# JunweiLiang/Multiverse

Measured on AMD Instinct MI355X. Metric: trajectories/sec (8-obs/12-pred, multi-scale 18x32+9x16 grid, greedy forward), higher is better.
Workload: dtype f16x3 (fp32 operands as two pre-scaled fp16 planes, fp32 accumulate and state; winograd F(3,3) over image rows on pre-transformed operands, 1.67 fp16 MFMAs issued per fp32 product over the gate kernels; error vs fp64 within 2x of the fp32-MFMA path's -- asserted under checkpoint-like dynamic range (; 1 GPU; BASELINE configs[1]: multi-scale 18x32+9x16 (scene 36x64x11), batch 64/GPU, fp32 forward-only, beam 1, obs 8 / pred 12; gate convolution on the fp16 matrix pipe (f16x3 split, fp32-class error); batch_per_gpu=64, global_batch=64, obs_len=8, pred_len=12, parallelism=batch-sharded x1, no data-path collective

## Files before the change

multiverse_amd/csrc/convlstm_mfma.h:

```cpp
#pragma once
#include <hip/hip_runtime.h>
#include <stdint.h>

#include <vector>

namespace mv {

typedef float f32x16 __attribute__((ext_vector_type(16)));
typedef float f32x4 __attribute__((ext_vector_type(4)));

constexpr int kBN = 128;
constexpr int kBK = 32;
constexpr int kChBlock = 32;
constexpr int kWaveRows = 32;
constexpr int kBlockRows = 128;
constexpr int kMaxGroup = 4;

struct ConvLstmArgs {
  const float* x;
  const float* h;
  const float* c;
  const int32_t* src_row_h;
  const int32_t* src_row_c;
  const float* wpack;
  const float* bias;
  float* h_out;
  float* c_out;
  float* gates_out;
  float* out0;
  float* out1;
  int32_t out0_cols, out1_cols;
  int32_t n_colblocks;
  int32_t ng_last;
  int32_t rows, H, W, Cx, C;
  int32_t x_row_stride;
  int32_t n_xchunks;
  int32_t n_hchunks;
  int32_t w_chunks;
  int32_t x_small;
  int32_t zero_state;
  float forget_bias;
  int32_t want_h16;
  int32_t skip_h32;
  const float* sx_bias;
  const float* sx_corr;
  const int32_t* sx_hot;
  const uint32_t* sx_cellyx;
  int32_t sx_hot_stride, sx_hot_div, sx_rad, sx_by_class;
  const int32_t* cone_list;
  const int32_t* cone_prev;
  int32_t cone_on;
  int32_t cone_cells;
};

struct ConvLstmGroup {
  ConvLstmArgs p[kMaxGroup];
  int32_t block_end[kMaxGroup];
  int32_t n;
};

static inline int convlstm_xchunks(int Cx) {
  if (Cx == 0) return 0;
  if (9 * Cx <= kBK) return 1;
  return 9 * (Cx / kBK);
}
static inline bool convlstm_cx_supported(int Cx) {
  return Cx == 0 || 9 * Cx <= kBK || (Cx % kBK) == 0;
}
static inline size_t convlstm_wpack_elems(int Cx, int C) {
  const size_t nch = (size_t)convlstm_xchunks(Cx) + 9 * (size_t)(C / kBK);
  return (size_t)(C / kChBlock) * nch * kBN * kBK;
}

static inline void pack_convlstm_weights(const float* w, int Cx, int C, float* out) {
  const int Cin = Cx + C, N4 = 4 * C;
  const int nx = convlstm_xchunks(Cx), nh = 9 * (C / kBK), nch = nx + nh;
  const bool small = (Cx > 0 && 9 * Cx <= kBK);
  for (int cb = 0; cb < C / kChBlock; ++cb)
    for (int q = 0; q < nch; ++q) {
      float* tile = out + ((size_t)cb * nch + q) * kBN * kBK;
      for (int kk = 0; kk < 4; ++kk)
        for (int g = 0; g < 4; ++g)
          for (int l = 0; l < 64; ++l)
            for (int j = 0; j < 4; ++j) {
              const int k = kk * 8 + (l >> 5) * 4 + j;
              const int n = g * C + cb * kChBlock + (l & 31);
              int tap = -1, ci = -1;
              if (q < nx) {
                if (small) {
                  if (k < 9 * Cx) { tap = k / Cx; ci = k % Cx; }
                } else {
                  tap = q % 9; ci = (q / 9) * kBK + k;
                }
              } else {
                const int qq = q - nx;
                tap = qq % 9; ci = Cx + (qq / 9) * kBK + k;
              }
              tile[((kk * 4 + g) * 64 + l) * 4 + j] =
                  (tap < 0) ? 0.f : w[((size_t)tap * Cin + ci) * N4 + n];
            }
    }
}

__device__ __forceinline__ float sigm_(float v) {
  const float e = __builtin_amdgcn_exp2f(-1.4426950408889634f * v);
// ... 301 lines not shown
```

multiverse_amd/csrc/convlstm_wino3.h:

```cpp
#pragma once
#include "convlstm_wino.h"

namespace mv {

template <int NRB>
struct Wn3 {
  static constexpr int kCh = 8 * NRB;
  static constexpr int kChunkVec = 5 * 3 * 2 * NRB * 64;
  static constexpr uint32_t kChunkBytes = kChunkVec * 16;
  static constexpr int kTileFloats = 96 * kCh;
};

static inline size_t wino3_wpack_elems(int Cx16, int C, int nrb) {
  return (size_t)(C / (8 * nrb)) * (size_t)(Cx16 / 16 + C / 16) * 5 * 3 * 2 * nrb * 64 * 8;
}

__global__ void pack_wino3_kernel(const float* __restrict__ w, _Float16* __restrict__ out,
                                  int Cx_total, int Cx16, int C, int nrb, size_t total) {
  const size_t idx = (size_t)blockIdx.x * blockDim.x + threadIdx.x;
  if (idx >= total) return;
  const int e = idx & 7;
  const int l = (idx >> 3) & 63;
  size_t t = idx >> 9;
  const int rb = (int)(t % nrb); t /= nrb;
// ... 15 lines not shown
  switch (comp) {
    case 0: u = 0.5 * g0; break;
    case 1: u = -0.5 * (g0 + g1 + g2); break;
    case 2: u = (-g0 + g1 - g2) / 6.0; break;
    case 3: u = (g0 + 2.0 * g1 + 4.0 * g2) / 6.0; break;
    default: u = -g2; break;
  }
  const double sv = u * 256.0;
  note_pack_range(sv);
  const _Float16 v0 = (_Float16)sv;
  const _Float16 v1 = (_Float16)(sv - (double)v0);
  const size_t vec = ((((size_t)cb * nch + chunk) * 5 + comp) * 3 + dx) * 2;
  out[(((vec + 0) * nrb + rb) * 64 + l) * 8 + e] = v0;
  out[(((vec + 1) * nrb + rb) * 64 + l) * 8 + e] = v1;
}

struct Wn3Consts { f16x8 m1, p2, m2; };

template <int KA, int KB>
__device__ __forceinline__ void wn_lin(const f16x8 a_hi, const f16x8 a_lo, const f16x8 b_hi,
                                       const f16x8 b_lo, const Wn3Consts& k, f16x8& hi,
                                       f16x8& lo) {
  static_assert((KA == 1 && (KB == 1 || KB == -1 || KB == -2)) || (KA == 2 && KB == 1), "form");
  const f16x8 nka = KA == 1 ? k.m1 : k.m2;
  f16x8 s, ne2, l1;
  if (KA == 2) {
    s = __builtin_elementwise_fma(a_hi, k.p2, b_hi);
    l1 = __builtin_elementwise_fma(a_lo, k.p2, b_lo);
  } else if (KB == 1) {
    s = a_hi + b_hi;
    l1 = a_lo + b_lo;
  } else {
    s = __builtin_elementwise_fma(b_hi, KB == -1 ? k.m1 : k.m2, a_hi);
    l1 = __builtin_elementwise_fma(b_lo, KB == -1 ? k.m1 : k.m2, a_lo);
  }
  const f16x8 bb = __builtin_elementwise_fma(a_hi, nka, s);
  const f16x8 t = __builtin_elementwise_fma(bb, k.m1, s);
  const f16x8 ne1 = __builtin_elementwise_fma(a_hi, nka, t);
  if (KB == -1) ne2 = bb + b_hi;
  else ne2 = __builtin_elementwise_fma(b_hi, KB == 1 ? k.m1 : k.p2, bb);
  hi = s;
  lo = __builtin_elementwise_fma(ne1 + ne2, k.m1, l1);
}

struct Wn3TransformItem {
  const _Float16* p0;
  int64_t pstride;
  _Float16* out;
  const int32_t* src_row;
  int32_t rows, H, W, Cc;
  const int32_t* cone_list;
  const int32_t* cone_prev;
  int32_t cone_cells;
};
constexpr int kW3TrGroup = 8;
struct Wn3TransformGroup {
  Wn3TransformItem it[kW3TrGroup];
  int32_t blk_end[kW3TrGroup];
  int32_t n;
};
static inline size_t wino3_v_elems(int rows, int H, int W, int Cc) {
  const size_t Q = (size_t)rows * ((H + 2) / 3) * W;
  return ((Q + 31) / 32) * (size_t)(Cc / 16) * 5 * 2 * 64 * 8;
}
static inline unsigned wino3_transform_blocks(int rows, int H, int W, int Cc) {
  const size_t Q = (size_t)rows * ((H + 2) / 3) * W;
  return (unsigned)((((Q + 31) / 32) * (size_t)(Cc / 16) + 3) / 4);
}
__global__ __launch_bounds__(256)
void wino3_transform_kernel(const Wn3TransformGroup g) {
  int block = blockIdx.x, pi = 0;
#pragma unroll
  for (int i = 0; i < kW3TrGroup - 1; ++i)
    if (i + 1 < g.n && (int)blockIdx.x >= g.blk_end[i]) pi = i + 1;
  if (pi > 0) block -= g.blk_end[pi - 1];
  const Wn3TransformItem& it = g.it[pi];
  const int lane = threadIdx.x & 63, wave = threadIdx.x >> 6;
  const int KG = it.Cc >> 4;
  const int H = it.H, W = it.W, HW = H * W;
  const int Kt = ((H + 2) / 3) * W, Q_total = it.rows * Kt;
  const int ntile = (Q_total + 31) >> 5;
  const int wid = block * 4 + wave;
  if (wid >= ntile * KG) return;
  int tile = wid / KG;
  const int cg = wid - tile * KG;
  if (it.cone_list) {
    if (tile >= it.cone_list[0]) return;
    tile = it.cone_list[4 + tile];
  }
  const int col = lane & 31, half = lane >> 5;
  const int q = tile * 32 + col;
  const bool valid = q < Q_total;
  int r = 0, y0 = 0, xpos = 0;
  if (valid) {
    r = q / Kt;
    const int pc = q - r * Kt;
    const int t = pc / W;
    y0 = 3 * t;
    xpos = pc - t * W;
  }
  const int sr = (valid && it.src_row) ? it.src_row[r] : r;
  int sr_up = sr, sr_mid = sr, sr_dn = sr;
  if (it.cone_prev && valid) {
    const int bg = it.rows - 1;
    const int* prev = it.cone_prev;
    sr_mid = prev[q >> 5] ? sr : bg;
    sr_up = (y0 > 0 && !prev[(q - W) >> 5]) ? bg : sr;
    sr_dn = (y0 + 3 < H && !prev[(q + W) >> 5]) ? bg : sr;
  }
  f16x8 dh[5], dl[5];
#pragma unroll
  for (int i = 0; i < 5; ++i) {
    const int rho = y0 - 1 + i;
    const bool ok = valid & (rho >= 0) & (rho < H);
    const long long m = (long long)(i == 0 ? sr_up : (i == 4 ? sr_dn : sr_mid)) * HW + rho * W + xpos;
    const size_t o = ((size_t)(m >> 5) * KG + cg) * 512 + (size_t)(half * 256 + (int)(m & 31) * 8);
    const f16x8 z = {0, 0, 0, 0, 0, 0, 0, 0};
    dh[i] = ok ? *reinterpret_cast<const f16x8*>(it.p0 + o) : z;
    dl[i] = ok ? *reinterpret_cast<const f16x8*>(it.p0 + it.pstride + o) : z;
  }
  uint32_t mone = 0xBC00BC00u, ptwo = 0x40004000u, mtwo = 0xC000C000u;
  asm volatile("" : "+s"(mone), "+s"(ptwo), "+s"(mtwo));
  Wn3Consts kc;
  kc.m1 = __builtin_bit_cast(f16x8, u32x4{mone, mone, mone, mone});
  kc.p2 = __builtin_bit_cast(f16x8, u32x4{ptwo, ptwo, ptwo, ptwo});
  kc.m2 = __builtin_bit_cast(f16x8, u32x4{mtwo, mtwo, mtwo, mtwo});
  f16x8 vh[5], vl[5], th, tl, t3h, t3l;
  wn_lin<1, -1>(dh[3], dl[3], dh[1], dl[1], kc, vh[3], vl[3]);
  wn_lin<1, -1>(dh[0], dl[0], dh[2], dl[2], kc, th, tl);
  wn_lin<2, 1>(th, tl, vh[3], vl[3], kc, vh[0], vl[0]);
  wn_lin<1, -1>(dh[3], dl[3], dh[2], dl[2], kc, t3h, t3l);
  wn_lin<1, -2>(t3h, t3l, dh[1], dl[1], kc, vh[1], vl[1]);
  wn_lin<1, -1>(dh[1], dl[1], dh[2], dl[2], kc, th, tl);
  wn_lin<2, 1>(th, tl, t3h, t3l, kc, vh[2], vl[2]);
  wn_lin<1, -1>(dh[2], dl[2], dh[4], dl[4], kc, th, tl);
  wn_lin<2, 1>(vh[3], vl[3], th, tl, kc, vh[4], vl[4]);
  f16x8* o = reinterpret_cast<f16x8*>(it.out) + ((size_t)tile * KG + cg) * (5 * 2 * 64) + lane;
#pragma unroll
  for (int c = 0; c < 5; ++c) {
    o[(c * 2 + 0) * 64] = vh[c];
    o[(c * 2 + 1) * 64] = vl[c];
  }
}
static inline void launch_wino3_transforms(const Wn3TransformItem* items, int n,
                                           hipStream_t stream) {
  for (int i0 = 0; i0 < n; i0 += kW3TrGroup) {
    Wn3TransformGroup g{};
    g.n = n - i0 < kW3TrGroup ? n - i0 : kW3TrGroup;
    unsigned nb = 0;
    for (int j = 0; j < g.n; ++j) {
      g.it[j] = items[i0 + j];
      nb += wino3_transform_blocks(g.it[j].rows, g.it[j].H, g.it[j].W, g.it[j].Cc);
      g.blk_end[j] = (int32_t)nb;
    }
    for (int j = g.n; j < kW3TrGroup; ++j) g.blk_end[j] = (int32_t)nb;
    if (nb) hipLaunchKernelGGL(wino3_transform_kernel, dim3(nb), dim3(256), 0, stream, g);
  }
}

template <int WAVES, int NRB, bool HALO, bool BF16D = false>
__device__ __forceinline__ void convlstm_wino3_body(const ConvLstmWinoArgs& p, int cb, int mt,
                                                    f16x8* lds) {
  using G = Wn3<NRB>;
  constexpr int CH = G::kCh;
  constexpr int kOwn = HALO ? 30 : 32;
  constexpr int kTriples = WAVES * kOwn;
  constexpr int kPieces = CH / 4;
  constexpr int kPasses = (96 * kPieces + 63) / 64;
  const ConvLstm16Args& q = p.b;
  const ConvLstmArgs& a = q.f;
  const int tid = threadIdx.x;
  const int lane = tid & 63;
// ... 371 lines not shown
        }
#pragma unroll
        for (int g = 0; g < 4; ++g)
          add[g] = *reinterpret_cast<const f32x4*>(bsrc + g * C + ch);
        if (a.sx_corr) {
          const int dy = y - hot_y, dxh = xpos - hot_x, rad = a.sx_rad;
          const bool inr = okc[e] && !bg_row && dy >= -rad && dy <= rad && dxh >= -rad && dxh <= rad;
          const int dyc = dy < -rad ? -rad : (dy > rad ? rad : dy);
          const int dxc = dxh < -rad ? -rad : (dxh > rad ? rad : dxh);
          const int side = 2 * rad + 1;
          const int idx = a.sx_by_class
                              ? 3 * (hot_y == 0 ? 0 : (hot_y == H - 1 ? 2 : 1)) +
                                    (hot_x == 0 ? 0 : (hot_x == W - 1 ? 2 : 1))
                              : ((valid && !bg_row) ? r : 0);
          const float* ct = a.sx_corr +
              ((size_t)idx * side * side + (dyc + rad) * side + (dxc + rad)) * 4 * C + ch;
          const float keep = inr ? 1.0f : 0.0f;
#pragma unroll
          for (int g = 0; g < 4; ++g) {
            const f32x4 cv = *reinterpret_cast<const f32x4*>(ct + g * C);
            add[g][0] = __builtin_fmaf(cv[0], keep, add[g][0]);
            add[g][1] = __builtin_fmaf(cv[1], keep, add[g][1]);
            add[g][2] = __builtin_fmaf(cv[2], keep, add[g][2]);
            add[g][3] = __builtin_fmaf(cv[3], keep, add[g][3]);
          }
        }
      }
      f32x4 cn4, hn4, si4, tj4, sf4, so4;
#pragma unroll
      for (int j = 0; j < 4; ++j) {
        float pre[4];
#pragma unroll
        for (int g = 0; g < 4; ++g) {
          const int reg = g * 4 + j;
          float yv;
          if constexpr (BF16D) {
            yv = acc[e][rb][reg];
          } else {
            const float m0 = acc[0][rb][reg], m1 = acc[1][rb][reg], m2 = acc[2][rb][reg],
                        m3 = acc[3][rb][reg], m4 = acc[kAcc - 1][rb][reg];
            if (e == 0) yv = (m0 + m1) + (m2 + m3);
            else if (e == 1) yv = (m1 - m2) + 2.0f * m3;
            else yv = (m1 + m2) + (4.0f * m3 + m4);
          }
          pre[g] = __builtin_fmaf(yv, un, add[g][j]);
        }
        const float si = sigm_(pre[0]), tj = tanh_(pre[1]), sf = sigm_(pre[2] + a.forget_bias),
                    so = sigm_(pre[3]);
        float cn = sf * cprev[e][rb][j];
        cn = cn + si * tj;
        const float hn = tanh_(cn) * so;
        cn4[j] = cn; hn4[j] = hn; si4[j] = si; tj4[j] = tj; sf4[j] = sf; so4[j] = so;
      }
      *reinterpret_cast<f32x4*>(tl0 + wr_idx + e * 32 * CH + rb * 8) = cn4;
      if (!a.skip_h32) *reinterpret_cast<f32x4*>(tl1 + wr_idx + e * 32 * CH + rb * 8) = hn4;
      if (a.gates_out && okc[e]) {
        const uint32_t g0 = (mcell * 4u * (uint32_t)C + (uint32_t)ch) * 4u;
        __builtin_amdgcn_raw_buffer_store_b128(__builtin_bit_cast(u32x4, si4), go_rs, (int)g0,
                                               0, MV_EPI_ST_AUX);
        __builtin_amdgcn_raw_buffer_store_b128(__builtin_bit_cast(u32x4, tj4), go_rs,
                                               (int)(g0 + rowb), 0, MV_EPI_ST_AUX);
        __builtin_amdgcn_raw_buffer_store_b128(__builtin_bit_cast(u32x4, sf4), go_rs,
                                               (int)(g0 + 2 * rowb), 0, MV_EPI_ST_AUX);
        __builtin_amdgcn_raw_buffer_store_b128(__builtin_bit_cast(u32x4, so4), go_rs,
                                               (int)(g0 + 3 * rowb), 0, MV_EPI_ST_AUX);
      }
      if (planes) {
        f16x4 p0, p1;
#pragma unroll
        for (int j = 0; j < 4; ++j) {
          if constexpr (BF16D) {
            p0[j] = bf16_as_half(hn4[j]);
            p1[j] = p0[j];
          } else {
            const float sc = hn4[j] * kF16Scale;
            const _Float16 h0 = (_Float16)sc;
            p0[j] = h0;
            p1[j] = (_Float16)(sc - (float)h0);
          }
        }
        ph[e][rb] = __builtin_bit_cast(u32x2, p0);
        pl[e][rb] = __builtin_bit_cast(u32x2, p1);
      }
    }
  }
  asm volatile("s_waitcnt lgkmcnt(0)" ::: "memory");
  {
#pragma unroll
    for (int k = 0; k < kPasses; ++k) {
      const int i = k * 64 + lane_e;
      const int trow = i / kPieces, piece = i - trow * kPieces;
      if (96 * kPieces % 64 == 0 || trow < 96) {
        const uint32_t ro = otab[96 + trow];
        const u32x4 cv = *reinterpret_cast<const u32x4*>(tl0 + i * 4);
        u32x4 hv = cv;
        if (!a.skip_h32) hv = *reinterpret_cast<const u32x4*>(tl1 + i * 4);
        if (ro != kNone) {
          const int off = (int)(ro + colb + (uint32_t)piece * 16u);
          __builtin_amdgcn_raw_buffer_store_b128(cv, co_rs, off, 0, MV_EPI_ST_AUX);
          if (!a.skip_h32) __builtin_amdgcn_raw_buffer_store_b128(hv, ho_rs, off, 0, MV_EPI_ST_AUX);
        }
      }
    }
  }
  if (planes) {
    const uint32_t mc01 = (uint32_t)(r * HW + (half_e ? cell[1] : cell[0]));
    const uint32_t mc2 = (uint32_t)(r * HW + cell[2]);
    const bool ok01 = half_e ? okc[1] : okc[0];
    const bool ok2 = okc[2] && half_e == 0;
    const size_t KG = (size_t)(C >> 4);
#pragma unroll
    for (int rb = 0; rb < NRB; ++rb) {
      const int c8 = cb * NRB + rb;
      const size_t grp = (size_t)(c8 >> 1) * 512 + (size_t)(c8 & 1) * 256;
      const size_t o01 = (size_t)(mc01 >> 5) * KG * 512 + grp + (size_t)((int)(mc01 & 31u) * 8);
      const size_t o2 = (size_t)(mc2 >> 5) * KG * 512 + grp + (size_t)((int)(mc2 & 31u) * 8);
#pragma unroll
      for (int pn = 0; pn < (BF16D ? 1 : 2); ++pn) {
        const u32x2 A = pn ? pl[0][rb] : ph[0][rb], B = pn ? pl[1][rb] : ph[1][rb];
        const u32x2 D = pn ? pl[2][rb] : ph[2][rb];
        const u32x2 s0 = __builtin_amdgcn_permlane32_swap(A[0], B[0], false, false);
        const u32x2 s1 = __builtin_amdgcn_permlane32_swap(A[1], B[1], false, false);
        const u32x4 v = {s0[0], s1[0], s0[1], s1[1]};
        if (ok01)
          *reinterpret_cast<u32x4*>(q.h16_out + (size_t)pn * q.h16_out_stride + o01) = v;
        const u32x2 t0 = __builtin_amdgcn_permlane32_swap(D[0], D[0], false, false);
        const u32x2 t1 = __builtin_amdgcn_permlane32_swap(D[1], D[1], false, false);
        const u32x4 v2 = {t0[0], t1[0], t0[1], t1[1]};
        if (ok2)
          *reinterpret_cast<u32x4*>(q.h16_out + (size_t)pn * q.h16_out_stride + o2) = v2;
      }
    }
  }
}

template <int WAVES, int NRB, bool HALO, bool BF16D = false>
__global__ __launch_bounds__(WAVES * 64, 2)
void convlstm_step_wino3_kernel(const ConvLstmWinoGroup g) {
  extern __shared__ __attribute__((aligned(16))) f16x8 lds[];
  int block = blockIdx.x;
  int pi = 0;
#pragma unroll
  for (int i = 0; i < kMaxGroup - 1; ++i)
    if (i + 1 < g.n && (int)blockIdx.x >= g.block_end[i]) pi = i + 1;
  if (pi > 0) block -= g.block_end[pi - 1];
  auto cbmap = [&](int ncb, int& cb, int& mt) {
    if ((g.map_mode == 2 || g.map_mode == 3) && ncb == 16) {
      const int per = g.map_mode == 2 ? 4 : 8;
      const int nt = per / 2;
      const int grp = block / (16 * nt), w = block - grp * (16 * nt);
      const int xcd = w & 7, j = w >> 3;
      cb = per * (xcd % (16 / per)) + j;
// ... 137 lines not shown
```

multiverse_amd/csrc/engine_forward.h:

```cpp
#pragma once

namespace {


using mv::ConvLstmArgs;

void set_sparse_x(mv_engine* e, ScaleState& S, ConvLstmArgs& a, bool decoder,
                  const int32_t* hot, int hot_stride, int hot_div) {
  a.sx_bias = decoder ? S.sx_dec_bias.p : nullptr;
  a.sx_corr = decoder ? S.sx_dec_corr.p : S.sx_enc_corr.p;
  a.sx_hot = hot; a.sx_hot_stride = hot_stride; a.sx_hot_div = hot_div;
  a.sx_cellyx = S.sx_cellyx.p;
  a.sx_rad = decoder ? 2 : 1;
  a.sx_by_class = decoder ? 1 : 0;
}

ConvLstmArgs conv_problem(mv_engine* e, const ConvCell& cc, const float* x,
                          const float* h, const float* c, const int32_t* src_row_h,
                          const int32_t* src_row_c, float* h_out, float* c_out,
                          int rows, int H, int W, bool zero_state,
                          size_t x_row_stride = 0, bool want_h16 = true) {
  ConvLstmArgs a{};
  const size_t xrs = x_row_stride ? x_row_stride : (size_t)H * W * cc.Cx;
  MV_REQUIRE((size_t)rows * H * W * e->cfg.hidden_size < ((size_t)1 << 31) &&
// ... 29 lines not shown
  throw HipError{"internal: unknown weight pack"};
}


void prepare_gate_operands(mv_engine* e, const std::vector<ConvLstmArgs>& probs,
                           const std::vector<ConvCell*>& cells,
                           std::vector<mv::ConvLstm16Args>& p16) {
  struct SplitItem { const float* in; _Float16* p0; _Float16* p1; int cells, C; };
  std::vector<SplitItem> splits;
  struct DynItem { const float* in; _Float16* p0; _Float16* p1; int cells, C; int32_t* bits; };
  std::vector<DynItem> dyn_splits;
  const bool bf16 = e->compute_mode == 2;
  auto ready = [&](const float* src) -> const mv_engine::PlaneBuf* {
    auto it = e->planes.find(src);
    return (it != e->planes.end() && it->second.valid) ? &it->second : nullptr;
  };
  for (size_t i = 0; i < probs.size(); ++i) {
    const ConvLstmArgs& a = probs[i];
    mv::ConvLstm16Args& q = p16[i];
    const size_t sl = (size_t)e->slot0 + i;
    MV_REQUIRE(a.H * a.W >= 32, "f16x3 / bf16 compute modes need grids of at least 32 cells "
               "(%d x %d); use compute mode f32", a.H, a.W);
    MV_REQUIRE((double)a.rows * a.H * a.W * a.C * 4.0 < 4294967296.0,
               "f16x3 / bf16 compute modes: state tensor of %d rows exceeds 4 GB", a.rows);
    MV_REQUIRE(!a.gates_out || (double)a.rows * a.H * a.W * a.C * 16.0 < 4294967296.0,
               "f16x3 / bf16 training forward: gate tensor of %d rows exceeds 4 GB "
               "(lower the per-GPU batch or use compute mode f32)", a.rows);
    q.f = a;
    q.wp16 = bf16 ? cells[i]->wpb.p : cells[i]->wp16.p;
    q.wx32 = bf16 ? cells[i]->wx32u.p : cells[i]->wx32.p;
    const size_t ncell = (size_t)a.rows * a.H * a.W;
    const size_t ncell_st = e->tl.issuing ? (size_t)e->cfg.batch_size * a.H * a.W : ncell;
    const int xpass = bf16_x_passes(e->compute_mode, e->dyn_x(), a.x_small);
    q.n_xk = a.x_small ? 0 : xpass * mv::f16x3_xksteps(a.Cx);
    q.n_hk = a.zero_state ? 0 : 9 * (a.C / 16);
    q.w_ksteps = (a.x_small ? 0 : xpass * mv::f16x3_xksteps(a.Cx)) + 9 * (a.C / 16);
    if (bf16)
      MV_REQUIRE((q.n_xk / 3) % MV_BF16_UNITS == 0 && (q.n_hk / 3) % MV_BF16_UNITS == 0,
                 "bf16 mode: %d x / %d h k-steps do not fill whole LDS stages (emb_size and "
                 "scene_conv_dim must be multiples of 32)", q.n_xk, q.n_hk);
    q.x16 = nullptr; q.h16 = nullptr;
    q.x_plane_stride = q.h_plane_stride = 0;
    q.h16_out = nullptr;
    q.h16_out_stride = 0;
    e->plane_invalidate(a.h_out);
    if (gate_knobs().epi_planes && a.want_h16 && !a.gates_out) {
      size_t pst = 0;
      if (_Float16* po = e->plane_out(a.h_out, &pst)) {
        q.h16_out = po;
        q.h16_out_stride = (int64_t)pst;
      }
    }
    q.f.skip_h32 = (a.skip_h32 && q.h16_out && !e->train) ? 1 : 0;
    if (has_dense_x(a)) {
      MV_REQUIRE((size_t)a.x_row_stride == (size_t)a.H * a.W * a.Cx,
                 "internal: f16x3 needs a contiguous x operand");
      if (const auto* pb = ready(a.x)) {
        q.x16 = pb->p; q.x_plane_stride = (int64_t)pb->n;
      } else {
        const size_t pst = ncell_st * a.Cx + mv::kPlaneSlack + mv::kPlanePad;
        MV_REQUIRE(e->px16[sl].n >= 2 * pst, "internal: f16x3 x plane scratch");
        _Float16* p0 = e->px16[sl].p + mv::kPlanePad;
        q.x16 = p0; q.x_plane_stride = (int64_t)pst;
        if (e->dyn_x()) {
          MV_REQUIRE(e->xexp[sl].p, "internal: x exponent scratch");
          q.x_exp = e->xexp[sl].p + 64;
          dyn_splits.push_back(DynItem{a.x, p0, p0 + pst, (int)ncell, a.Cx, e->xexp[sl].p});
        } else {
          splits.push_back(SplitItem{a.x, p0, bf16 ? (_Float16*)nullptr : p0 + pst, (int)ncell, a.Cx});
        }
      }
      MV_REQUIRE(!(bf16 && e->dyn_x()) || q.x_exp, "internal: bf16 mode, unbounded activations: "
                 "a dense x operand came as producer planes, without its exponent");
    }
    if (!a.zero_state) {
      if (const auto* pb = ready(a.h)) {
        q.h16 = pb->p; q.h_plane_stride = (int64_t)pb->n;
      } else {
        const size_t pst = ncell_st * a.C + mv::kPlaneSlack + mv::kPlanePad;
        MV_REQUIRE(e->ph16[sl].n >= 2 * pst, "internal: f16x3 h plane scratch");
        _Float16* p0 = e->ph16[sl].p + mv::kPlanePad;
        q.h16 = p0; q.h_plane_stride = (int64_t)pst;
        splits.push_back(SplitItem{a.h, p0, bf16 ? (_Float16*)nullptr : p0 + pst, (int)ncell, a.C});
      }
    }
  }
  for (const DynItem& it : dyn_splits) {
    launch(e, "split_planes", 0, 12.0 * (double)it.cells * it.C, [&] {
      HIP_CHECK(hipMemsetAsync(it.bits, 0, 64 * sizeof(int32_t), e->issue));
      hipLaunchKernelGGL(mv::absmax_bits_kernel, dim3(256), dim3(256), 0, e->issue, it.in,
                         (size_t)it.cells * it.C, it.bits);
      hipLaunchKernelGGL(mv::split_planes_dyn_kernel,
                         dim3(mv::split_planes_blocks((size_t)it.cells, it.C)), dim3(256), 0,
                         e->issue, it.in, it.p0, it.p1, it.cells, it.C, it.bits, it.bits + 64);
    });
  }
  for (size_t s0 = 0; s0 < splits.size(); s0 += mv::kSplitGroup) {
    mv::SplitGroup g{};
    double sbytes = 0;
    unsigned nb = 0;
    g.n = (int)std::min<size_t>(mv::kSplitGroup, splits.size() - s0);
    for (int j = 0; j < g.n; ++j) {
      const SplitItem& it = splits[s0 + j];
      g.in[j] = it.in; g.p0[j] = it.p0; g.p1[j] = it.p1; g.M[j] = it.cells; g.C[j] = it.C;
      nb += mv::split_planes_blocks((size_t)it.cells, it.C);
      g.blk_end[j] = nb;
      sbytes += (bf16 ? 6.0 : 8.0) * (double)it.cells * it.C;
    }
    launch(e, "split_planes", 0, sbytes, [&] {
      hipLaunchKernelGGL(mv::split_planes_group_kernel, dim3(nb), dim3(256), 0, e->issue, g);
    });
  }
}

double queue_wino3_transform(std::vector<mv::Wn3TransformItem>& tr, const mv::Wn3TransformItem& it) {
  tr.push_back(it);
  const double cells = it.cone_cells ? (double)it.cone_cells : (double)it.rows * it.H * it.W;
  return cells * it.Cc * 4.0 * (1.0 + 5.0 / 3.0);
}

void launch_gate_group(const ForwardPlan& pl, const mv::ConvLstm16Args* p16,
                       const _Float16* const* packs, const float* const* w_hwio,
                       _Float16* const* v3x, _Float16* const* v3h, int n, hipStream_t stream) {
  if (pl.form == GateForm::Direct16)
    return mv::launch_convlstm16_steps(p16, n, pl.shift, pl.map_mode, stream);
  if (pl.form == GateForm::Bf16)
    return mv::launch_convlstm_bf16_steps(p16, n, pl.shift, pl.map_mode, pl.x_passes == 3, stream);
  mv::ConvLstmWinoArgs pw[mv::kMaxGroup] = {};
  for (int i = 0; i < n; ++i) {
    pw[i].b = p16[i];
    pw[i].wpw = packs[i];
    pw[i].w_hwio = w_hwio[i];
    pw[i].n_xc = p16[i].f.x_small ? 0 : p16[i].f.Cx / 16;
    pw[i].v3x = v3x ? v3x[i] : nullptr;
    pw[i].v3h = v3h ? v3h[i] : nullptr;
  }
  if (pl.form == GateForm::Wino2) mv::launch_convlstm_wino_steps(pw, n, pl.map_mode, stream);
  else if (pl.form == GateForm::Wino3)
// ... 15 lines not shown
  for (const auto& a : probs) {
    const double Md = (double)(a.rows - (a.cone_on ? 1 : 0)) * a.H * a.W;
    const double M = a.cone_cells ? (double)a.cone_cells : (double)a.rows * a.H * a.W;
    dense += 2.0 * Md * 9.0 * (a.Cx + a.C) * 4.0 * a.C;
    const double cx = a.sx_corr ? 0.0 : (double)a.Cx;
    flops += 2.0 * M * 9.0 * (cx + (a.zero_state ? 0 : a.C)) * 4.0 * a.C;
    bytes += M * (cx + (a.zero_state ? 2.0 : 4.0) * a.C) * 4.0;
  }
}

GatePrep prepare_gate_group(mv_engine* e, const std::vector<ConvLstmArgs>& probs) {
  GatePrep g;
  const int n = (int)probs.size();
  MV_REQUIRE(e->slot0 + n <= mv::kMaxGroup, "internal: gate group of %d problems from slot %d",
             n, e->slot0);
  g.slot0 = e->slot0;
  g.cells.resize(n);
  for (int i = 0; i < n; ++i) g.cells[i] = cell_of_pack(e, probs[i].wpack);
  g.p16.resize(n);
  prepare_gate_operands(e, probs, g.cells, g.p16);
  gate_group_cost(probs, g.flops, g.bytes, g.dense);
  return g;
}

ForwardPlan plan_gate_groups(mv_engine* e, const GatePrep* const* groups, int ngroups) {
  ForwardProblem fp[mv::kMaxGroup];
  int n = 0;
  for (int g = 0; g < ngroups; ++g)
    for (int i = 0; i < groups[g]->n(); ++i) {
      MV_REQUIRE(n < mv::kMaxGroup, "internal: more than %d gate problems in a step", mv::kMaxGroup);
      const int sl = groups[g]->slot0 + i;
      fp[n++] = ForwardProblem{&groups[g]->p16[i], groups[g]->cells[i], e->pv3x[sl].n, e->pv3h[sl].n};
    }
  const ForwardPlan pl = plan_forward_group(e->compute_mode, fp, n);
  check_cone_plan(pl, fp, n);
  return pl;
}

void issue_gate_group(mv_engine* e, const GatePrep& g, const ForwardPlan& pl) {
  const int n = g.n();
  const _Float16* packs[mv::kMaxGroup] = {};
  const float* w_hwio[mv::kMaxGroup] = {};
  _Float16 *v3x[mv::kMaxGroup] = {}, *v3h[mv::kMaxGroup] = {};
  std::vector<mv::Wn3TransformItem> tr3;
  double tr3_bytes = 0;
  for (int i = 0; i < n; ++i) {
    const mv::ConvLstm16Args& q = g.p16[i];
    const ConvLstmArgs& a = q.f;
    const int sl = g.slot0 + i;
    w_hwio[i] = g.cells[i]->kernel->dev.p;
    packs[i] = pl.form == GateForm::Wino2 ? g.cells[i]->wpw.p
             : pl.form == GateForm::Wino3 ? g.cells[i]->wpw3.p
             : pl.form == GateForm::Bf16T ? g.cells[i]->wpbt.p : nullptr;
    if (pl.form != GateForm::Wino3) continue;
    if (!a.zero_state) {
      v3h[i] = e->pv3h[sl].p;
      tr3_bytes += queue_wino3_transform(tr3, {q.h16, q.h_plane_stride, v3h[i], a.src_row_h,
                                               a.rows, a.H, a.W, a.C, a.cone_list, a.cone_prev,
                                               a.cone_cells});
    }
    if (has_dense_x(a)) {
      v3x[i] = e->pv3x[sl].p;
      tr3_bytes += queue_wino3_transform(tr3, {q.x16, q.x_plane_stride, v3x[i], nullptr,
                                               a.rows, a.H, a.W, a.Cx});
    }
  }
  if (!tr3.empty())
    launch(e, "wino3_transform", 0, tr3_bytes, [&] {
      mv::launch_wino3_transforms(tr3.data(), (int)tr3.size(), e->issue);
    });
  for (int i = 0; i < n; ++i)
    e->gate_rows += g.p16[i].f.rows - (g.p16[i].f.cone_on ? 1 : 0);
  launch(e, "convlstm_step", g.flops, g.bytes, [&] {
    launch_gate_group(pl, g.p16.data(), packs, w_hwio, v3x, v3h, n, e->issue);
  }, g.dense, pl.mfma_factor);
}

void run_conv_group_f16x3(mv_engine* e, const std::vector<ConvLstmArgs>& probs) {
  const GatePrep g = prepare_gate_group(e, probs);
  const GatePrep* gp = &g;
  issue_gate_group(e, g, plan_gate_groups(e, &gp, 1));
}

void run_conv_group(mv_engine* e, const std::vector<ConvLstmArgs>& probs) {
  if (probs.empty()) return;
  if (e->compute_mode != 0) {
    run_conv_group_f16x3(e, probs);
    return;
  }
  double flops = 0, bytes = 0, dense = 0;
  gate_group_cost(probs, flops, bytes, dense);
  for (const auto& a : probs) e->gate_rows += a.rows;
  if (e->cfg.convlstm_kernel != 3) {
    const double kk = (double)e->cfg.convlstm_kernel * e->cfg.convlstm_kernel / 9.0;
    launch(e, "convlstm_step", flops * kk, bytes, [&] {
      for (const auto& a : probs) {
        mv::ConvGenericArgs ga{};
        ga.f = a;
        ga.w = cell_of_bias(e, a.bias)->kernel->dev.p;
        ga.ksize = e->cfg.convlstm_kernel;
        mv::launch_convlstm_generic_step(ga, e->issue);
      }
    }, dense * kk, 0.0);
    return;
  }
  launch(e, "convlstm_step", flops, bytes, [&] {
    mv::launch_convlstm_steps(probs.data(), (int)probs.size(), e->issue);
  }, dense, 1.0);
}

void run_conv_pairs(mv_engine* e, const std::vector<ConvLstmArgs>& a,
                    const std::vector<ConvLstmArgs>& b) {
// ... 452 lines not shown
    if (!pl.do_reg) continue;
    mv::TailProblem b = tail_problem(S.q_reg.p, pl.reg_out, pl.reg_stride, reg_rows, S.H, S.W,
                                     false, E, c.activation);
    tbytes += 4.0 * cr * (18 + 2);
    if (pl.reg_next) {
      if (pl.reg_x_out) {
        tail_embed(b, S.emb_reg_W->dev.p, S.emb_reg_b->dev.p, pl.reg_x_out);
        tbytes += 4.0 * cr * E;
      } else {
        size_t pst = 0;
        _Float16* x16 = e->plane_out(S.xbuf_reg.p, &pst);
        tail_embed(b, S.emb_reg_W->dev.p, S.emb_reg_b->dev.p, S.xbuf_reg.p, x16, pst);
        tbytes += 4.0 * cr * E * (b.x16 ? 2 : 1);
      }
    }
    tp.push_back(b);
  }
  MV_REQUIRE(qp.size() <= (size_t)mv::kTailMax, "decode tail: too many chains");
  if (qp.empty()) return;
  launch(e, "hidden2grid", qflops, qbytes, [&] {
    mv::launch_h2g_q(qp.data(), (int)qp.size(), C, e->issue);
  });
  launch(e, "decode_tail", 0, tbytes, [&] {
    mv::launch_decode_tail(tp.data(), (int)tp.size(), e->issue);
  });
}

void tail_reg_chain(const ScaleState& S, const Cursors& cur, int s, int t, int Tp, int rows,
                    TailPlan& pl) {
  pl.reg_h = S.reg_h[cur.reg[s]].p;
  pl.reg_out = S.out_reg.p + (size_t)t * S.K * 2; pl.reg_stride = (int64_t)Tp * S.K * 2;
  pl.reg_next = t + 1 < Tp;
  pl.reg_rows = rows;
}

ConvLstmArgs beam_cls_problem(mv_engine* e, int s, Cursors& cur, int time, int rows,
                              const int32_t* src_h, const int32_t* src_c, int first_div,
                              const int32_t* prev_ids, int prev_stride) {
  const mv_config& c = e->cfg;
  ScaleState& S = e->sc[s];
  const int cc = cur.cls[s], T = c.obs_len;
  const float* hin = c.use_gnn ? S.cls_hg.p : S.cls_h[cc].p;
  ConvLstmArgs a = conv_problem(e, S.dec_cls, S.xbuf_cls.p, hin, S.cls_c[cc].p, src_h, src_c,
                                S.cls_h[cc ^ 1].p, S.cls_c[cc ^ 1].p, rows, S.H, S.W, false, 0,
                                !c.use_gnn);
  if (sparse_x_on(e, S)) {
    if (time == 1) set_sparse_x(e, S, a, true, S.labels.p + (T - 1), T, first_div);
    else set_sparse_x(e, S, a, true, prev_ids, prev_stride, 1);
  }
  cur.cls[s] ^= 1;
  return a;
}

void run_decoders_greedy(mv_engine* e, Cursors& cur, int Tp, bool pairs) {
  const mv_config& c = e->cfg;
  const int T = c.obs_len;
  const bool v2 = tail_grouped(e);
  MV_REQUIRE(!pairs || (v2 && !c.use_single_decoder), "internal: chain pairs need the grouped "
             "decoder tail and a regression decoder");
  const int Tsteps = e->len.ragged ? e->len.steps : Tp;
  for (int t = 0; t < Tsteps; ++t) {
    const int N = e->rows_at(t);
    auto step_problems = [&](int chains, std::vector<ConvLstmArgs>& probs) {
      if ((chains & kChainCls) && c.use_gnn) {
        std::vector<GnnJob> jobs;
        for (int s = 0; s < c.num_scales; ++s)
          if (e->sc[s].use)
            jobs.push_back(GnnJob{&e->sc[s], e->sc[s].cls_h[cur.cls[s]].p, nullptr,
                                  e->sc[s].cls_hg.p, N, 1});
        run_gnn_jobs(e, jobs);
      }
      for (int s = 0; s < c.num_scales; ++s) {
        ScaleState& S = e->sc[s];
        if (!S.use) continue;
        if (chains & kChainCls) {
          const int cc = cur.cls[s];
          const float* hin = c.use_gnn ? S.cls_hg.p : S.cls_h[cc].p;
          const bool sparse = sparse_x_on(e, S) && (t == 0 || !c.class_feedback_dense);
          if (sparse)
            ;
          else if (t == 0)
            run_emb_onehot(e, S, S.labels.p + (T - 1), T, S.xbuf_cls.p, N);
          else if (c.class_feedback_dense)
            run_emb_dense(e, S, S.out_cls.p + (size_t)(t - 1) * S.K, (size_t)Tp * S.K,
                          S.xbuf_cls.p, N, S.emb_cls_W, S.emb_cls_b, 1);
          else if (!v2)
            run_emb_onehot(e, S, S.ids.p, 1, S.xbuf_cls.p, N);
          probs.push_back(conv_problem(e, S.dec_cls, S.xbuf_cls.p, hin, S.cls_c[cc].p,
                                       nullptr, nullptr, S.cls_h[cc ^ 1].p,
                                       S.cls_c[cc ^ 1].p, N, S.H, S.W, false, 0,
                                       !c.use_gnn));
          if (sparse) {
            if (t == 0) set_sparse_x(e, S, probs.back(), true, S.labels.p + (T - 1), T, 1);
            else set_sparse_x(e, S, probs.back(), true, S.ids.p, 1, 1);
          }
          cur.cls[s] ^= 1;
        }
        if ((chains & kChainReg) && !c.use_single_decoder)
          probs.push_back(reg_decoder_problem(e, s, cur, t, Tp, !v2));
      }
      std::stable_sort(probs.begin(), probs.end(), [](const ConvLstmArgs& a, const ConvLstmArgs& b) {
        return (a.sx_corr == nullptr) > (b.sx_corr == nullptr);
      });
    };
    auto step_tail = [&](int chains) {
      std::vector<TailPlan> plans;
      for (int s = 0; s < c.num_scales; ++s) {
        ScaleState& S = e->sc[s];
        if (!S.use) continue;
        TailPlan pl{};
        pl.s = s;
        pl.cls_h = S.cls_h[cur.cls[s]].p; pl.cls_rows = N;
        pl.cls_out = S.out_cls.p + (size_t)t * S.K; pl.cls_stride = (int64_t)Tp * S.K;
        pl.cls_next = t + 1 < Tp && !c.class_feedback_dense;
        tail_reg_chain(S, cur, s, t, Tp, N, pl);
        if (c.use_single_decoder) {
          pl.reg_h = pl.cls_h;
          pl.reg_next = false;
        }
        pl.do_cls = (chains & kChainCls) != 0;
        pl.do_reg = (chains & kChainReg) != 0;
        plans.push_back(pl);
      }
      run_tail(e, plans);
    };
    if (pairs) {
      std::vector<ConvLstmArgs> pa, pb;
      { IssueOn on(e, 0); step_problems(kChainCls, pa); }
      { IssueOn on(e, 1); step_problems(kChainReg, pb); }
      run_conv_pairs(e, pa, pb);
      { IssueOn on(e, 0); step_tail(kChainCls); }
      { IssueOn on(e, 1); step_tail(kChainReg); }
      continue;
    }
    std::vector<ConvLstmArgs> probs;
    step_problems(kChainAll, probs);
    run_conv_group(e, probs);
    if (v2) {
      step_tail(kChainAll);
      continue;
    }
    for (int s = 0; s < c.num_scales; ++s) {
      ScaleState& S = e->sc[s];
      if (!S.use) continue;
      const size_t orow = (size_t)Tp * S.K;
      float* logits = S.out_cls.p + (size_t)t * S.K;
      run_hidden2grid<1>(e, S, S.cls_h[cur.cls[s]].p, S.out_cls_W->dev.p, logits, orow, N);
      if (t + 1 < Tp && !c.class_feedback_dense) {
        launch(e, "argmax_rows", 0, 4.0 * N * S.K, [&] {
          hipLaunchKernelGGL(mv::argmax_rows_kernel, dim3(N), dim3(64), 0, e->issue,
                             logits, orow, S.ids.p, N, S.K);
        });
// ... 576 lines not shown
```

multiverse_amd/csrc/gate_plan.h:

```cpp
#pragma once

namespace {

struct GateKnobs {
  bool wino, wino3, bf16t, wino_dgrad;
  int wino_map_f23;
  int wino_map_f33;
  int wino_map_bf16t;
  bool conv_shift;
  int conv_map;
  bool epi_planes;
  int dgrad_kslices;
  bool transpose3;
  bool bf16_bwd;
  bool bf16_fused_split;
  bool wgrad_splits_set; int wgrad_splits;
  bool wgrad_wide;
  int wgrad_wide_map;
  int wgrad_wide_splits;
  bool wgrad_wide_x;
  bool wgrad_wino, wgrad_wino_bf16;
  int wgrad_x_splits;
  int enc_cone;
};

inline int env_num(const char* name, int unset) {
  const char* v = getenv(name);
  return v ? atoi(v) : unset;
}
inline bool env_on(const char* name) { return env_num(name, 1) != 0; }

inline const GateKnobs& gate_knobs() {
  static const GateKnobs k = [] {
    const auto num = env_num;
    const auto on = env_on;
    GateKnobs g{};
    g.wino = on("MV_WINO"); g.wino3 = on("MV_WINO3"); g.bf16t = on("MV_BF16T");
    g.wino_dgrad = on("MV_WINO_DGRAD");
    g.wino_map_f23 = num("MV_WINO_MAP", 1);
    g.wino_map_f33 = num("MV_WINO_MAP", 2);
    g.wino_map_bf16t = num("MV_WINO_MAP", 2);
    g.conv_shift = on("MV_CONV_SHIFT");
    g.conv_map = num("MV_CONV_MAP", 0);
    g.epi_planes = on("MV_EPI_PLANES");
    g.dgrad_kslices = num("MV_DGRAD_KSLICES", 0);
    g.transpose3 = on("MV_TRANSPOSE3");
    g.bf16_bwd = on("MV_BF16_BWD");
    g.bf16_fused_split = on("MV_BF16_FUSED_SPLIT");
    g.wgrad_splits_set = getenv("MV_WGRAD_SPLITS") != nullptr;
    g.wgrad_splits = num("MV_WGRAD_SPLITS", 0);
    g.wgrad_wide = on("MV_WGRAD_WIDE");
    g.wgrad_wide_map = num("MV_WGRAD_WIDE_MAP", 0);
    g.wgrad_wide_splits = num("MV_WGRAD_WIDE_SPLITS", 0);
    g.wgrad_wide_x = num("MV_WGRAD_WIDE_X", 0) == 1;
    g.wgrad_wino = on("MV_WGRAD_WINO"); g.wgrad_wino_bf16 = on("MV_WGRAD_WINO_BF16");
    g.wgrad_x_splits = num("MV_WGRAD_X_SPLITS", 12);
    g.enc_cone = num("MV_ENC_CONE", 1);
    return g;
  }();
  return k;
}

inline bool x_is_small(int Cx) { return Cx > 0 && 9 * Cx <= mv::kBK; }
inline int x_chunk16(int Cx) { return x_is_small(Cx) ? 0 : Cx; }
inline int bf16_x_passes(int mode, bool dyn_x, bool x_small) {
  return (mode == 2 && dyn_x && !x_small) ? 3 : 1;
}

struct CellPacks {
  bool wp16, wpw, wpw3;
  bool wpb, wpbt;
  bool wd16, wdw, wdb;
};
inline CellPacks cell_packs(int mode, int activation, int Cx, int C, bool wino_numerics_ok) {
  const GateKnobs& k = gate_knobs();
  const bool blocks_ok = C % mv::kWnCh == 0 && (Cx % 16 == 0 || x_is_small(Cx));
  CellPacks p{};
  p.wp16 = mode == 1;
  p.wpw = mode == 1 && k.wino && blocks_ok && wino_numerics_ok;
  p.wpw3 = p.wpw && k.wino3;
  p.wpb = mode == 2;
  p.wpbt = mode == 2 && k.bf16t && blocks_ok && activation == 0;
  p.wdb = mode == 2 && k.bf16_bwd;
  p.wd16 = mode != 0 && !p.wdb;
  p.wdw = p.wd16 && mode == 1 && k.wino && k.wino_dgrad;
  return p;
}

inline size_t wino3_scratch_elems(int rows, int H, int W, int Cc) {
  return H < 3 ? 0 : mv::wino3_v_elems(rows, H, W, (Cc + 15) / 16 * 16);
}
inline bool wino3_possible(int mode, int activation) {
  return mode == 1 && gate_knobs().wino && gate_knobs().wino3 && activation == 0;
}

constexpr int kEncConeMinBatch = 16;
inline bool enc_cone_geometry(int obs_len, int H, int W, int batch) {
  const int k = gate_knobs().enc_cone;
  return k != 0 && (k == 2 || batch >= kEncConeMinBatch) && obs_len >= 3 && H % 3 == 0 &&
         H / 3 >= 5 && W == 32;
}
inline bool cone_step_member_ok(int H, int W, bool has_packs) {
  return H >= 3 && W > 0 && 32 % W == 0 && has_packs;
}
inline bool enc_cone_planned(int mode, int activation, bool sparse, bool step_exact, int obs_len,
                             int H, int W, int C, int batch) {
  return enc_cone_geometry(obs_len, H, W, batch) && sparse && step_exact &&
         wino3_possible(mode, activation) && C % mv::kWnCh == 0;
}
inline int enc_cone_tiles(int rows, int H, int W) { return (rows * ((H + 2) / 3) * W + 31) / 32; }
// ... 19 lines not shown

inline ForwardPlan plan_forward_group(int mode, const ForwardProblem* p, int n) {
  const GateKnobs& k = gate_knobs();
  ForwardPlan pl;
  bool halo = false, halo_ok = true, shift = k.conv_shift, x_exp = false;
  for (int i = 0; i < n; ++i) {
    const mv::ConvLstmArgs& a = p[i].q->f;
    halo = halo || mv::wino3_needs_halo(a);
    halo_ok = halo_ok && mv::wino3_halo_addressable(a);
    shift = shift && a.W > 0 && 32 % a.W == 0;
    x_exp = x_exp || p[i].q->x_exp != nullptr;
  }
  const bool tile3_ok = !halo || halo_ok;
  bool wino = mode == 1 && k.wino, wino3 = wino && k.wino3 && tile3_ok;
  bool bf16t = mode == 2 && k.bf16t && tile3_ok;
  for (int i = 0; i < n; ++i) {
    const mv::ConvLstm16Args& q = *p[i].q;
    const mv::ConvLstmArgs& a = q.f;
    wino = wino && mv::wino_geometry_ok(a) && p[i].cell->wpw.p;
    wino3 = wino3 && mv::wino3_geometry_ok(a, q) && p[i].cell->wpw3.p &&
            (a.zero_state || p[i].v3h_cap >= wino3_scratch_elems(a.rows, a.H, a.W, a.C)) &&
            (!has_dense_x(a) || p[i].v3x_cap >= wino3_scratch_elems(a.rows, a.H, a.W, a.Cx));
    bf16t = bf16t && mv::bf16t_geometry_ok(a, q) && p[i].cell->wpbt.p;
  }
  pl.shift = shift;
  pl.map_mode = k.conv_map;
  if (mode == 2) {
    pl.form = bf16t ? GateForm::Bf16T : GateForm::Bf16;
    pl.mfma_factor = 1.0;
    if (bf16t) { pl.halo = halo; pl.map_mode = k.wino_map_bf16t; }
    else pl.x_passes = x_exp ? 3 : 1;
    return pl;
  }
  if (!wino && !wino3) return pl;
  pl.form = wino3 ? GateForm::Wino3 : GateForm::Wino2;
  pl.halo = wino3 && halo;
  pl.map_mode = wino3 ? k.wino_map_f33 : k.wino_map_f23;
  double num = 0, den = 0;
  for (int i = 0; i < n; ++i) {
    const mv::ConvLstmArgs& a = p[i].q->f;
    const double cx = a.sx_corr ? 0.0 : (double)a.Cx;
    const double fl = (double)a.rows * a.H * a.W * (cx + (a.zero_state ? 0 : a.C));
    const double per = wino3 ? 5.0 * ((a.H + 2) / 3) / a.H * (mv::wino3_needs_halo(a) ? 32.0 / 30.0 : 1.0)
                             : 4.0 * ((a.H + 1) / 2) / a.H;
    num += fl * per; den += fl;
  }
  pl.mfma_factor = den > 0 ? num / den : (wino3 ? 5.0 / 3.0 : 2.0);
  return pl;
}
inline void check_cone_plan(const ForwardPlan& pl, const ForwardProblem* p, int n) {
  for (int i = 0; i < n; ++i)
    MV_REQUIRE(!p[i].q->f.cone_on || (pl.form == GateForm::Wino3 && !pl.halo),
               "internal: a coned class-encoder step was planned outside the exact F(3,3) tiling");
}

struct DgradPlan {
  bool bf16 = false;
  bool wino = false;
  bool shift = false;
  double mfma_factor = 3.0;
  struct Slices { int nks_main, nks_x, n_kslice; } s[mv::kMaxGroup];
};
inline bool wino_dgrad_geometry_ok(const mv::ConvLstmArgs& a) {
  return a.W > 0 && 32 % a.W == 0 && a.H >= 2 && a.out0_cols % 64 == 0 && (a.C / 16) % 8 == 0;
}
inline DgradPlan plan_dgrad_group(int mode, const mv::ConvLstmArgs* probs, const bool* has_wdw,
                                  int n) {
  const GateKnobs& k = gate_knobs();
  DgradPlan pl;
  pl.bf16 = mode == 2 && k.bf16_bwd;
  pl.wino = mode == 1 && k.wino && k.wino_dgrad;
  pl.shift = k.conv_shift;
  for (int i = 0; i < n; ++i) {
    pl.wino = pl.wino && wino_dgrad_geometry_ok(probs[i]) && has_wdw[i];
    pl.shift = pl.shift && probs[i].W > 0 && 32 % probs[i].W == 0;
  }
  pl.mfma_factor = pl.wino ? 2.0 : (pl.bf16 ? 1.0 : 3.0);
  for (int i = 0; i < n; ++i) {
    const mv::ConvLstmArgs& a = probs[i];
    DgradPlan::Slices& s = pl.s[i];
    s = DgradPlan::Slices{0, 0, 0};
    if (pl.wino) {
      const int ncm = a.out0_cols / 64;
      int nkm = std::max(1, 8 / ncm);
      while ((a.C / 16) % nkm != 0) nkm /= 2;
      s.nks_main = nkm;
      s.nks_x = (a.out1 && a.out1_cols > 0) ? 8 : 1;
      continue;
    }
    const int nstages = 9 * (a.C / 16) / 3;
    const int ks = k.dgrad_kslices > 0 ? k.dgrad_kslices : (pl.bf16 ? 1 : 4);
    if (pl.bf16)
      MV_REQUIRE(nstages % MV_BF16_UNITS == 0, "internal: bf16 dgrad stage count %d", nstages);
    if (ks > 1 && nstages % (2 * ks) == 0) s.n_kslice = ks;
  }
  return pl;
}

struct WgradPlan {
  bool generic = false;
  bool f16 = false;
  bool one = false;
  bool wino = false;
  bool wide = false;
  bool wide_x = false;
  bool transpose3 = true;
// ... 48 lines not shown
```

Measured before the change: 4391 trajectories/sec.

## Read fp32 h directly in wino3 transform and skip last-step state stores

The F(3,3) input transform gains a path that loads the previous step's fp32 hidden state, splits it into scaled fp16 hi/lo planes in registers, and reorders lanes with ds_bpermute. Decoder steps can then stop emitting the fp16 h planes and skip the separate split_planes pass. The final greedy decoder step also skips the cell-state and fp16-h stores that nothing reads afterward. This removes memory traffic and kernel launches per decoder step, at the cost of more register and permute work inside the transform kernel and more complex plan conditions.

After: 4406 trajectories/sec (median of 6 runs). Within noise of the previous version (+0.3%).

```diff
diff --git a/multiverse_amd/csrc/convlstm_mfma.h b/multiverse_amd/csrc/convlstm_mfma.h
--- a/multiverse_amd/csrc/convlstm_mfma.h
+++ b/multiverse_amd/csrc/convlstm_mfma.h
@@ -51,6 +51,8 @@
   const int32_t* cone_prev;
   int32_t cone_on;
   int32_t cone_cells;
+  int32_t skip_c_out;
+  int32_t h_from_fp32;
 };
 
 struct ConvLstmGroup {
diff --git a/multiverse_amd/csrc/convlstm_wino3.h b/multiverse_amd/csrc/convlstm_wino3.h
--- a/multiverse_amd/csrc/convlstm_wino3.h
+++ b/multiverse_amd/csrc/convlstm_wino3.h
@@ -91,6 +91,8 @@
   const int32_t* cone_list;
   const int32_t* cone_prev;
   int32_t cone_cells;
+  const float* h32;
+  int64_t h32_row_stride;
 };
 constexpr int kW3TrGroup = 8;
 struct Wn3TransformGroup {
@@ -106,6 +108,7 @@
   const size_t Q = (size_t)rows * ((H + 2) / 3) * W;
   return (unsigned)((((Q + 31) / 32) * (size_t)(Cc / 16) + 3) / 4);
 }
+static inline bool wino3_transform_fp32_ok(int Cc) { return Cc % 16 == 0; }
 __global__ __launch_bounds__(256)
 void wino3_transform_kernel(const Wn3TransformGroup g) {
   int block = blockIdx.x, pi = 0;
@@ -148,6 +151,65 @@
     sr_dn = (y0 + 3 < H && !prev[(q + W) >> 5]) ? bg : sr;
   }
   f16x8 dh[5], dl[5];
+  if (it.h32) {
+    const int chunk = lane & 3;
+    f32x4 v[2][5];
+#pragma unroll
+    for (int j = 0; j < 2; ++j) {
+      const int qj = tile * 32 + (lane >> 2) + 16 * j;
+      const bool vj = qj < Q_total;
+      int rj = 0, yj = 0, xj = 0;
+      if (vj) {
+        rj = qj / Kt;
+        const int pc = qj - rj * Kt;
+        const int tt = pc / W;
+        yj = 3 * tt;
+        xj = pc - tt * W;
+      }
+      const int srj = (vj && it.src_row) ? it.src_row[rj] : rj;
+#pragma unroll
+      for (int i = 0; i < 5; ++i) {
+        const int rho = yj - 1 + i;
+        const bool ok = vj & (rho >= 0) & (rho < H);
+        const f32x4 z4 = {0.f, 0.f, 0.f, 0.f};
+        const float* s = it.h32 + (size_t)srj * (size_t)it.h32_row_stride +
+                         (size_t)(ok ? rho * W + xj : 0) * (size_t)it.Cc + (size_t)(cg * 16 + chunk * 4);
+        v[j][i] = ok ? *reinterpret_cast<const f32x4*>(s) : z4;
+      }
+    }
+    const int src_b = (4 * (col & 15) + 2 * half) * 4;
+    const bool upper = col >= 16;
+#pragma unroll
+    for (int i = 0; i < 5; ++i) {
+      u32x2 ph[2], pl[2];
+#pragma unroll
+      for (int j = 0; j < 2; ++j) {
+        f16x4 p0, p1;
+#pragma unroll
+        for (int k = 0; k < 4; ++k) {
+          const float sc = v[j][i][k] * kF16Scale;
+          const _Float16 h0 = (_Float16)sc;
+          p0[k] = h0;
+          p1[k] = (_Float16)(sc - (float)h0);
+        }
+        ph[j] = __builtin_bit_cast(u32x2, p0);
+        pl[j] = __builtin_bit_cast(u32x2, p1);
+      }
+      u32x4 oh, ol;
+#pragma unroll
+      for (int d = 0; d < 4; ++d) {
+        const int sa = src_b + (d >> 1) * 4;
+        const uint32_t h0 = (uint32_t)__builtin_amdgcn_ds_bpermute(sa, (int)ph[0][d & 1]);
+        const uint32_t h1 = (uint32_t)__builtin_amdgcn_ds_bpermute(sa, (int)ph[1][d & 1]);
+        const uint32_t l0 = (uint32_t)__builtin_amdgcn_ds_bpermute(sa, (int)pl[0][d & 1]);
+        const uint32_t l1 = (uint32_t)__builtin_amdgcn_ds_bpermute(sa, (int)pl[1][d & 1]);
+        oh[d] = upper ? h1 : h0;
+        ol[d] = upper ? l1 : l0;
+      }
+      dh[i] = __builtin_bit_cast(f16x8, oh);
+      dl[i] = __builtin_bit_cast(f16x8, ol);
+    }
+  } else {
 #pragma unroll
   for (int i = 0; i < 5; ++i) {
     const int rho = y0 - 1 + i;
@@ -157,6 +219,7 @@
     const f16x8 z = {0, 0, 0, 0, 0, 0, 0, 0};
     dh[i] = ok ? *reinterpret_cast<const f16x8*>(it.p0 + o) : z;
     dl[i] = ok ? *reinterpret_cast<const f16x8*>(it.p0 + it.pstride + o) : z;
+  }
   }
   uint32_t mone = 0xBC00BC00u, ptwo = 0x40004000u, mtwo = 0xC000C000u;
   asm volatile("" : "+s"(mone), "+s"(ptwo), "+s"(mtwo));
@@ -634,7 +697,7 @@
         const float hn = tanh_(cn) * so;
         cn4[j] = cn; hn4[j] = hn; si4[j] = si; tj4[j] = tj; sf4[j] = sf; so4[j] = so;
       }
-      *reinterpret_cast<f32x4*>(tl0 + wr_idx + e * 32 * CH + rb * 8) = cn4;
+      if (!a.skip_c_out) *reinterpret_cast<f32x4*>(tl0 + wr_idx + e * 32 * CH + rb * 8) = cn4;
       if (!a.skip_h32) *reinterpret_cast<f32x4*>(tl1 + wr_idx + e * 32 * CH + rb * 8) = hn4;
       if (a.gates_out && okc[e]) {
         const uint32_t g0 = (mcell * 4u * (uint32_t)C + (uint32_t)ch) * 4u;
@@ -674,12 +737,13 @@
       const int trow = i / kPieces, piece = i - trow * kPieces;
       if (96 * kPieces % 64 == 0 || trow < 96) {
         const uint32_t ro = otab[96 + trow];
-        const u32x4 cv = *reinterpret_cast<const u32x4*>(tl0 + i * 4);
+        u32x4 cv = {0u, 0u, 0u, 0u};
+        if (!a.skip_c_out) cv = *reinterpret_cast<const u32x4*>(tl0 + i * 4);
         u32x4 hv = cv;
         if (!a.skip_h32) hv = *reinterpret_cast<const u32x4*>(tl1 + i * 4);
         if (ro != kNone) {
           const int off = (int)(ro + colb + (uint32_t)piece * 16u);
-          __builtin_amdgcn_raw_buffer_store_b128(cv, co_rs, off, 0, MV_EPI_ST_AUX);
+          if (!a.skip_c_out) __builtin_amdgcn_raw_buffer_store_b128(cv, co_rs, off, 0, MV_EPI_ST_AUX);
           if (!a.skip_h32) __builtin_amdgcn_raw_buffer_store_b128(hv, ho_rs, off, 0, MV_EPI_ST_AUX);
         }
       }
diff --git a/multiverse_amd/csrc/engine_forward.h b/multiverse_amd/csrc/engine_forward.h
--- a/multiverse_amd/csrc/engine_forward.h
+++ b/multiverse_amd/csrc/engine_forward.h
@@ -105,6 +105,8 @@
       }
     }
     q.f.skip_h32 = (a.skip_h32 && q.h16_out && !e->train) ? 1 : 0;
+    q.f.skip_c_out = (a.skip_c_out && !a.gates_out && !e->train) ? 1 : 0;
+    bool from_fp32 = false;
     if (has_dense_x(a)) {
       MV_REQUIRE((size_t)a.x_row_stride == (size_t)a.H * a.W * a.Cx,
                  "internal: f16x3 needs a contiguous x operand");
@@ -134,9 +136,11 @@
         MV_REQUIRE(e->ph16[sl].n >= 2 * pst, "internal: f16x3 h plane scratch");
         _Float16* p0 = e->ph16[sl].p + mv::kPlanePad;
         q.h16 = p0; q.h_plane_stride = (int64_t)pst;
-        splits.push_back(SplitItem{a.h, p0, bf16 ? (_Float16*)nullptr : p0 + pst, (int)ncell, a.C});
-      }
-    }
+        if (a.h_from_fp32 && !a.src_row_h && !e->train) from_fp32 = true;
+        else splits.push_back(SplitItem{a.h, p0, bf16 ? (_Float16*)nullptr : p0 + pst, (int)ncell, a.C});
+      }
+    }
+    q.f.h_from_fp32 = from_fp32 ? 1 : 0;
   }
   for (const DynItem& it : dyn_splits) {
     launch(e, "split_planes", 0, 12.0 * (double)it.cells * it.C, [&] {
@@ -258,12 +262,25 @@
     packs[i] = pl.form == GateForm::Wino2 ? g.cells[i]->wpw.p
              : pl.form == GateForm::Wino3 ? g.cells[i]->wpw3.p
              : pl.form == GateForm::Bf16T ? g.cells[i]->wpbt.p : nullptr;
+    const bool h_fp32 = a.h_from_fp32 && pl.form == GateForm::Wino3 && !pl.halo && !a.cone_on &&
+                        mv::wino3_transform_fp32_ok(a.C);
+    if (a.h_from_fp32 && !h_fp32) {
+      const size_t ncell = (size_t)a.rows * a.H * a.W;
+      launch(e, "split_planes", 0, 8.0 * (double)ncell * a.C, [&] {
+        hipLaunchKernelGGL(mv::split_planes_kernel, dim3(mv::split_planes_blocks(ncell, a.C)),
+                           dim3(256), 0, e->issue, a.h, const_cast<_Float16*>(q.h16),
+                           e->compute_mode == 2 ? (_Float16*)nullptr
+                                                : const_cast<_Float16*>(q.h16) + q.h_plane_stride,
+                           (int)ncell, a.C);
+      });
+    }
     if (pl.form != GateForm::Wino3) continue;
     if (!a.zero_state) {
       v3h[i] = e->pv3h[sl].p;
-      tr3_bytes += queue_wino3_transform(tr3, {q.h16, q.h_plane_stride, v3h[i], a.src_row_h,
-                                               a.rows, a.H, a.W, a.C, a.cone_list, a.cone_prev,
-                                               a.cone_cells});
+      mv::Wn3TransformItem it{q.h16, q.h_plane_stride, v3h[i], a.src_row_h, a.rows, a.H, a.W, a.C,
+                              a.cone_list, a.cone_prev, a.cone_cells};
+      if (h_fp32) { it.h32 = a.h; it.h32_row_stride = (int64_t)a.H * a.W * a.C; }
+      tr3_bytes += queue_wino3_transform(tr3, it);
     }
     if (has_dense_x(a)) {
       v3x[i] = e->pv3x[sl].p;
@@ -822,10 +839,33 @@
   return a;
 }
 
+bool decoders_exact_w3(mv_engine* e) {
+  const mv_config& c = e->cfg;
+  bool ok = c.hidden_size % mv::kWnCh == 0;
+  for (int s = 0; s < c.num_scales; ++s) {
+    ScaleState& S = e->sc[s];
+    if (!S.use) continue;
+    ok = ok && cone_step_member_ok(S.H, S.W, S.dec_cls.wpw3.p != nullptr &&
+                                   (c.use_single_decoder || S.dec_reg.wpw3.p != nullptr));
+  }
+  return ok;
+}
+
 void run_decoders_greedy(mv_engine* e, Cursors& cur, int Tp, bool pairs) {
   const mv_config& c = e->cfg;
   const int T = c.obs_len;
   const bool v2 = tail_grouped(e);
+  const bool h_fp32 = wino3_h_from_fp32(e->compute_mode, c.activation, e->train,
+                                        decoders_exact_w3(e), false);
+  const bool last_skips = last_step_skips_stores(e->compute_mode, e->train, e->len.ragged,
+                                                 c.class_feedback_dense != 0);
+  auto trim_stores = [&](ConvLstmArgs& a, bool chain_fp32, int t, int Tsteps) {
+    if (chain_fp32) {
+      a.h_from_fp32 = t > 0 ? 1 : 0;
+      if (t + 1 < Tsteps) a.want_h16 = 0;
+    }
+    if (last_skips && t + 1 == Tsteps) { a.want_h16 = 0; a.skip_c_out = 1; }
+  };
   MV_REQUIRE(!pairs || (v2 && !c.use_single_decoder), "internal: chain pairs need the grouped "
              "decoder tail and a regression decoder");
   const int Tsteps = e->len.ragged ? e->len.steps : Tp;
@@ -864,10 +904,13 @@
             if (t == 0) set_sparse_x(e, S, probs.back(), true, S.labels.p + (T - 1), T, 1);
             else set_sparse_x(e, S, probs.back(), true, S.ids.p, 1, 1);
           }
+          trim_stores(probs.back(), h_fp32 && !c.use_gnn, t, Tsteps);
           cur.cls[s] ^= 1;
         }
-        if ((chains & kChainReg) && !c.use_single_decoder)
+        if ((chains & kChainReg) && !c.use_single_decoder) {
           probs.push_back(reg_decoder_problem(e, s, cur, t, Tp, !v2));
+          trim_stores(probs.back(), h_fp32, t, Tsteps);
+        }
       }
       std::stable_sort(probs.begin(), probs.end(), [](const ConvLstmArgs& a, const ConvLstmArgs& b) {
         return (a.sx_corr == nullptr) > (b.sx_corr == nullptr);
diff --git a/multiverse_amd/csrc/gate_plan.h b/multiverse_amd/csrc/gate_plan.h
--- a/multiverse_amd/csrc/gate_plan.h
+++ b/multiverse_amd/csrc/gate_plan.h
@@ -22,6 +22,8 @@
   bool wgrad_wino, wgrad_wino_bf16;
   int wgrad_x_splits;
   int enc_cone;
+  bool tr_fp32;
+  bool last_step_stores;
 };
 
 inline int env_num(const char* name, int unset) {
@@ -56,6 +58,8 @@
     g.wgrad_wino = on("MV_WGRAD_WINO"); g.wgrad_wino_bf16 = on("MV_WGRAD_WINO_BF16");
     g.wgrad_x_splits = num("MV_WGRAD_X_SPLITS", 12);
     g.enc_cone = num("MV_ENC_CONE", 1);
+    g.tr_fp32 = on("MV_TR_FP32");
+    g.last_step_stores = num("MV_LAST_STEP_STORES", 0) != 0;
     return g;
   }();
   return k;
@@ -181,6 +185,15 @@
   for (int i = 0; i < n; ++i)
     MV_REQUIRE(!p[i].q->f.cone_on || (pl.form == GateForm::Wino3 && !pl.halo),
                "internal: a coned class-encoder step was planned outside the exact F(3,3) tiling");
+}
+
+inline bool wino3_h_from_fp32(int mode, int activation, bool train, bool next_exact_w3,
+                              bool skip_h32) {
+  return gate_knobs().tr_fp32 && !train && wino3_possible(mode, activation) && next_exact_w3 &&
+         !skip_h32;
+}
+inline bool last_step_skips_stores(int mode, bool train, bool ragged, bool class_feedback_dense) {
+  return !gate_knobs().last_step_stores && mode == 1 && !train && !ragged && !class_feedback_dense;
 }
 
 struct DgradPlan {
```
